# xingyizhou/CenterTrack

Hardware: NVIDIA H100
Metric: frames/sec (device-timed) DLA-34 512x512 (higher is better)
Workload: dtype bf16

## Files before the change

centertrack_b200/_lib.py:

```python
import ctypes as C
import os
import subprocess

_HERE = os.path.dirname(os.path.abspath(__file__))
LIB_PATH = os.path.join(_HERE, 'libctb200.so')
CSRC = os.path.join(_HERE, 'csrc')
SOURCES = ['api.cu', 'conv_simt.cu', 'conv_tc.cu', 'conv_halo.cu', 'elementwise.cu', 'decode.cu', 'stream.cu']

CT_F32, CT_BF16 = 0, 1
CT_A_CONV, CT_A_DCN, CT_A_DCN_WIN = 0, 1, 2
CT_OUT_NHWC, CT_OUT_NHWC_F32, CT_OUT_NCHW_F32, CT_OUT_NHWC_S2D = 0, 1, 2, 3
CT_HEAD_NONE, CT_HEAD_SIGMOID, CT_HEAD_DEPTH = 0, 1, 2
CT_ENGINE_SIMT, CT_ENGINE_TCGEN05, CT_ENGINE_TCGEN05_HALO, CT_ENGINE_TCGEN05_X3 = 0, 1, 2, 3
CT_ROLE_RAW, CT_ROLE_REG, CT_ROLE_WH, CT_ROLE_LTRB, CT_ROLE_LTRB_AMODAL, CT_ROLE_HPS = range(6)
CT_DECODE_MAX_HEADS = 12
CT_REC_SCORE, CT_REC_CLS, CT_REC_XS, CT_REC_YS, CT_REC_BBOX, CT_REC_IND, CT_REC_HEADS = 0, 1, 2, 3, 4, 8, 9


class ConvDesc(C.Structure):
  _fields_ = [
      ('engine', C.c_int32), ('dtype', C.c_int32), ('a_mode', C.c_int32),
      ('B', C.c_int32), ('H', C.c_int32), ('W', C.c_int32),
      ('C_in', C.c_int32), ('ld_in', C.c_int32), ('C_out', C.c_int32),
      ('KH', C.c_int32), ('KW', C.c_int32), ('stride', C.c_int32), ('pad', C.c_int32),
      ('OH', C.c_int32), ('OW', C.c_int32), ('ld_out', C.c_int32), ('out_mode', C.c_int32),
      ('relu', C.c_int32), ('ld_res', C.c_int32), ('head_act', C.c_int32),
      ('sig_from', C.c_int32), ('depth_scale', C.c_float), ('ld_om', C.c_int32),
      ('n_tile', C.c_int32), ('epilogue_sum3', C.c_int32), ('pad_w1', C.c_int32),
      ('x', C.c_void_p), ('w', C.c_void_p), ('shift', C.c_void_p), ('residual', C.c_void_p),
      ('om', C.c_void_p), ('out', C.c_void_p),
  ]


class DecodeHead(C.Structure):
  _fields_ = [('map', C.c_void_p), ('channels', C.c_int32), ('role', C.c_int32),
              ('rec_offset', C.c_int32)]


class DecodeDesc(C.Structure):
  _fields_ = [
# ... 19 lines not shown
      ('records', C.c_void_p), ('trans_out_inv', C.c_void_p), ('trans_input', C.c_void_p),
      ('tracks', C.c_void_p), ('counts', C.c_void_p), ('boxes', C.c_void_p),
  ]


class TrackAssoc(C.Structure):
  _fields_ = [
      ('hungarian', C.c_int32), ('public_det', C.c_int32), ('max_public', C.c_int32),
      ('public_ct', C.c_void_p), ('public_n', C.c_void_p), ('steps', C.c_void_p),
  ]


class TrackPayload(C.Structure):
  _fields_ = [
      ('width', C.c_int32), ('payload', C.c_void_p), ('rec_hps', C.c_int32), ('hps_floats', C.c_int32),
      ('rec_dep', C.c_int32), ('rec_dim', C.c_int32), ('rec_rot', C.c_int32), ('rec_amodel_offset', C.c_int32),
      ('rec_velocity', C.c_int32), ('velocity_floats', C.c_int32), ('rec_nuscenes_att', C.c_int32),
      ('att_floats', C.c_int32), ('calib', C.c_void_p),
  ]


EXPORTS = ['ct_packed_weight_bytes', 'ct_pack_weights', 'ct_conv_forward', 'ct_stem_forward',
           'ct_pack_stem_input', 'ct_pack_stem_input_f32', 'ct_maxpool2', 'ct_maxpool2_s2d', 'ct_upsample_add', 'ct_decode_workspace_bytes', 'ct_decode',
           'ct_render_pre_hm', 'ct_track_smem_bytes', 'ct_track_step', 'ct_track_assoc_smem_bytes',
           'ct_track_step_assoc', 'ct_track_payload_smem_bytes', 'ct_track_step_payload', 'ct_render_tracks', 'ct_flip_merge',
           'ct_warp_affine_normalize', 'ct_last_error', 'ct_abi_version', 'ct_launch_count',
           'ct_reset_launch_count', 'ct_debug_trace', 'ct_debug_watch']

NVCC_FLAGS = ['-gencode', 'arch=compute_90a,code=sm_90a', '-lineinfo', '-O3', '-std=c++17', '-Xcompiler', '-fPIC']


def build(force=False, verbose=False):
  srcs = [os.path.join(CSRC, s) for s in SOURCES]
  deps = srcs + [os.path.join(CSRC, h) for h in ('common.cuh', 'conv_common.cuh', 'ptx.cuh', 'wgmma.cuh')] + \
      [os.path.join(_HERE, '..', 'include', 'ctb200.h')]
  if not force and os.path.exists(LIB_PATH) and \
      all(os.path.getmtime(LIB_PATH) >= os.path.getmtime(d) for d in deps):
    return LIB_PATH
  import shutil
  import tempfile
  with tempfile.TemporaryDirectory(prefix='ctb_build_') as tmp:
    objs = [os.path.join(tmp, os.path.basename(s) + '.o') for s in srcs]
    procs = [subprocess.Popen(['nvcc'] + NVCC_FLAGS + (['-Xptxas', '-v'] if verbose else []) + ['-c', s, '-o', o],
                              stdout=subprocess.PIPE, stderr=subprocess.STDOUT, text=True)
             for s, o in zip(srcs, objs)]
    logs = [p.communicate()[0] for p in procs]
    for s, p, log in zip(srcs, procs, logs):
      if p.returncode != 0:
        raise RuntimeError('nvcc failed on %s:\n%s' % (os.path.basename(s), log))
    if verbose:
      print(''.join(logs))
    tmp_lib = os.path.join(tmp, 'libctb200.so')
    r = subprocess.run(['nvcc', '-gencode', 'arch=compute_90a,code=sm_90a', '-shared', '-o', tmp_lib] + objs,
                       capture_output=True, text=True)
    if r.returncode != 0:
      raise RuntimeError('nvcc link failed:\n' + r.stdout + r.stderr)
    shutil.move(tmp_lib, LIB_PATH)
  return LIB_PATH


_lib = None


def lib():
  global _lib
  if _lib is not None:
    return _lib
# ... 56 lines not shown
```

centertrack_b200/csrc/api.cu:

```cuda
#include "conv_common.cuh"
#include <vector>

namespace ctb {
thread_local char g_err[512] = {0};
thread_local int64_t g_launches = 0;

static inline uint16_t f32_to_bf16_rn(float f) {
  uint32_t u;
  memcpy(&u, &f, 4);
  if ((u & 0x7fffffffu) > 0x7f800000u) return (uint16_t)((u >> 16) | 0x40);
  const uint32_t lsb = (u >> 16) & 1u;
  u += 0x7fffu + lsb;
  return (uint16_t)(u >> 16);
}
}

using namespace ctb;

extern "C" const char* ct_last_error(void) { return g_err; }
extern "C" int ct_abi_version(void) { return CTB200_ABI_VERSION; }
extern "C" int64_t ct_launch_count(void) { return g_launches; }
extern "C" void ct_reset_launch_count(void) { g_launches = 0; }
extern "C" int ct_debug_trace(void* device_buf) {
  const int r = halo_set_trace(device_buf);
  return r != CT_OK ? r : tc_set_trace(device_buf);
}
extern "C" int ct_debug_watch(void* mapped_host_buf) {
  int r = halo_set_watch(mapped_host_buf);
  if (r == CT_OK) r = tc_set_watch(mapped_host_buf);
  if (r == CT_OK) r = decode_set_watch(mapped_host_buf);
  return r;
}

static inline int tc_k_slices(int C_in, int KH, int KW) { return (KH * KW * C_in + 63) / 64; }

extern "C" int64_t ct_packed_weight_bytes(int32_t engine, int32_t C_out, int32_t C_in, int32_t KH,
                                          int32_t KW, int32_t n_tile) {
  if (engine == CT_ENGINE_SIMT) {
    const int64_t ldw = (C_out + 63) / 64 * 64;
    return (int64_t)KH * KW * C_in * ldw * 4;
  }
  if (n_tile <= 0 || n_tile % 16 != 0 || n_tile > 256) return -1;
  const int64_t n_tiles = (C_out + n_tile - 1) / n_tile;
  if (engine == CT_ENGINE_TCGEN05_HALO) {
    if (!(C_in == 8 || (C_in % 16 == 0 && C_in <= 64) || (C_in % 64 == 0 && C_in <= 256))) return -1;
    return n_tiles * halo_blocks(C_in, KH, KW) * (int64_t)n_tile * 32;
  }
  return n_tiles * tc_k_slices(C_in, KH, KW) * (int64_t)n_tile * 64 * 2 * (engine == CT_ENGINE_TCGEN05_X3 ? 2 : 1);
}

extern "C" int ct_pack_weights(int32_t engine, const float* w, int32_t C_out, int32_t C_in, int32_t KH,
                               int32_t KW, int32_t n_tile, void* dst) {
  CT_REQUIRE(w && dst, "null pointer");
  CT_REQUIRE(C_out > 0 && C_in > 0 && KH > 0 && KW > 0, "bad shape");
  const int taps = KH * KW;
  if (engine == CT_ENGINE_SIMT) {
    const int ldw = (C_out + 63) / 64 * 64;
    float* o = (float*)dst;
    memset(o, 0, (size_t)taps * C_in * ldw * 4);
    for (int oc = 0; oc < C_out; ++oc)
      for (int c = 0; c < C_in; ++c)
        for (int t = 0; t < taps; ++t)
          o[((size_t)t * C_in + c) * ldw + oc] = w[((size_t)oc * C_in + c) * taps + t];
// ... 88 lines not shown
```

centertrack_b200/csrc/conv_common.cuh:

```cuda
#pragma once
#include "common.cuh"
#include <cudaTypedefs.h>
#include <type_traits>

namespace ctb {

struct ConvGeom {
  int B, H, W, C_in, ld_in;
  int C_out, KH, KW, stride, pad, pad_w, OH, OW;
  int ld_out, out_mode, relu, ld_res, head_act, sig_from;
  float depth_scale;
  int ld_om;
  int P_out;
  int K_total;
};

inline ConvGeom make_geom(const ct_conv_desc* d) {
  ConvGeom g;
  g.B = d->B; g.H = d->H; g.W = d->W; g.C_in = d->C_in; g.ld_in = d->ld_in;
  g.C_out = d->C_out; g.KH = d->KH; g.KW = d->KW; g.stride = d->stride; g.pad = d->pad;
  g.pad_w = d->pad_w1 > 0 ? d->pad_w1 - 1 : d->pad;
  g.OH = d->OH; g.OW = d->OW; g.ld_out = d->ld_out; g.out_mode = d->out_mode;
  g.relu = d->relu; g.ld_res = d->ld_res; g.head_act = d->head_act; g.sig_from = d->sig_from;
  g.depth_scale = d->depth_scale; g.ld_om = d->ld_om;
// ... 43 lines not shown
                    q == cudaDriverEntryPointSuccess;
    return ok ? reinterpret_cast<PFN_cuTensorMapEncodeTiled>(p) : nullptr;
  }();
  if (!encode) return fail(CT_ERR_CUDA, "cuTensorMapEncodeTiled entry point unavailable%s", "");
  const cuuint32_t estr[5] = {1, 1, 1, 1, 1};
  const CUresult cr = encode(map, CU_TENSOR_MAP_DATA_TYPE_BFLOAT16, (cuuint32_t)rank, const_cast<void*>(ptr), dims,
                             strides, box, estr, CU_TENSOR_MAP_INTERLEAVE_NONE, swizzle,
                             CU_TENSOR_MAP_L2_PROMOTION_L2_128B, CU_TENSOR_MAP_FLOAT_OOB_FILL_NONE);
  return cr == CUDA_SUCCESS ? CT_OK : fail(CT_ERR_CUDA, "cuTensorMapEncodeTiled failed%s (%ld)", "", (long)cr);
}

template <auto Kernel, typename... Args>
int launch_big_smem(dim3 grid, dim3 block, size_t smem, cudaStream_t st, const Args&... args) {
  int dev = 0;
  cudaGetDevice(&dev);
  static thread_local unsigned long long attr_set_mask = 0;
  if (dev >= 64 || !((attr_set_mask >> dev) & 1ull)) {
    CT_CUDA_OK(cudaFuncSetAttribute(Kernel, cudaFuncAttributeMaxDynamicSharedMemorySize, 227 * 1024));
    if (dev < 64) attr_set_mask |= 1ull << dev;
  }
  CT_CUDA_OK(launch_kernel(Kernel, grid, block, smem, st, true, args...));
  return after_launch();
}

template <int N = 16, typename F>
int dispatch_n_tile(int n_tile, F&& f) {
  if constexpr (N > 256) return fail(CT_ERR_INVALID, "unsupported n_tile%s (%ld)", "", (long)n_tile);
  else return n_tile == N ? f(std::integral_constant<int, N>()) : dispatch_n_tile<N + 16>(n_tile, f);
}

int conv_forward_simt(const ct_conv_desc* d, cudaStream_t st);
int conv_forward_tc(const ct_conv_desc* d, cudaStream_t st);
int conv_forward_halo(const ct_conv_desc* d, cudaStream_t st);
int halo_blocks(int C_in, int KH, int KW);
int halo_set_trace(void* buf);
int tc_set_trace(void* buf);
int halo_set_watch(void* mapped_host_buf);
int tc_set_watch(void* mapped_host_buf);
int decode_set_watch(void* mapped_host_buf);

}
```

centertrack_b200/csrc/conv_tc.cu:

```cuda
#include "conv_common.cuh"
#include "wgmma.cuh"
#include <cuda.h>
#include <stdlib.h>

namespace ctb {

constexpr int TC_BM = 128;
constexpr int TC_BK = 64;
constexpr int TC_THREADS = 256;
constexpr int TC_PRODUCERS = 256;
constexpr int TC_NROW = TC_BM * 8 / TC_PRODUCERS;
constexpr int A_STAGE_BYTES = TC_BM * 128;

struct TcArgs {
  ConvGeom g;
  const __nv_bfloat16* x;
  const __nv_bfloat16* w;
  const float* shift;
  const __nv_bfloat16* residual;
  const float* om;
  void* out;
  int n_tile, k_slices, stages, a_mode;
  int tiles_x, tiles_y;
  int win_m, win_pw, win_ph;
  uint32_t win_bytes;
  uint32_t region0;
};

struct __align__(16) DcnWinEntry { int goff; uint32_t meta; uint32_t w01, w23; };
constexpr uint32_t WIN_DX = 1u << 16, WIN_DY = 1u << 17, WIN_IN = 1u << 18;

__device__ __forceinline__ int tc_pixel(const TcArgs& a, int mt, int r) {
  const ConvGeom& g = a.g;
  if (a.tiles_x == 0) { const int p = mt * TC_BM + r; return p < g.P_out ? p : g.P_out; }
  const int tpi = a.tiles_x * a.tiles_y;
  const int b = mt / tpi, t = mt - b * tpi;
  const int ty = t / a.tiles_x, tx = t - ty * a.tiles_x;
  const int oy = ty * 8 + (r >> 4), ox = tx * 16 + (r & 15);
  return (oy < g.OH && ox < g.OW) ? (b * g.OH + oy) * g.OW + ox : g.P_out;
}

__device__ unsigned long long* g_tc_trace = nullptr;
__device__ __forceinline__ unsigned long long* tc_trace_ptr() {
  unsigned long long* t = g_tc_trace;
  return (t != nullptr && blockIdx.x == gridDim.x / 2 && blockIdx.y == 0) ? t : nullptr;
}
__device__ __forceinline__ void tc_stamp(unsigned long long* t, int k) {
  if (t != nullptr && k < 256) t[k] = (unsigned long long)clock64();
}

__device__ __forceinline__ uint64_t make_sdesc(uint32_t smem_addr) {
  return wg_desc(smem_addr, 16u, 1024u, 1u);
}

struct __align__(16) DcnEntry { int off, dxo, dyo, pad; float w00, w01, w10, w11; };

struct DcnCorner { int y0, x0, yc, xc; bool dx, dy; float w00, w01, w10, w11; };
__device__ __forceinline__ bool dcn_corner(float py, float px, int H, int W, float m, DcnCorner& c) {
  if (!(py > -1.f && py < (float)H && px > -1.f && px < (float)W)) return false;
  const float y0f = floorf(py), x0f = floorf(px);
  const int y0 = (int)y0f, x0 = (int)x0f;
  const float ly = py - y0f, lx = px - x0f, hy = 1.f - ly, hx = 1.f - lx;
  const bool y0ok = y0 >= 0, y1ok = y0 + 1 <= H - 1, x0ok = x0 >= 0, x1ok = x0 + 1 <= W - 1;
  c.y0 = y0; c.x0 = x0; c.yc = max(y0, 0); c.xc = max(x0, 0);
  c.dx = x0ok && x1ok; c.dy = y0ok && y1ok;
  c.w00 = (y0ok && x0ok) ? hy * hx * m : 0.f;
  c.w01 = (y0ok && x1ok) ? hy * lx * m : 0.f;
  c.w10 = (y1ok && x0ok) ? ly * hx * m : 0.f;
  c.w11 = (y1ok && x1ok) ? ly * lx * m : 0.f;
  return true;
}

__device__ __forceinline__ uint32_t bmul2(uint32_t a, uint32_t b) {
  uint32_t d;
  asm("mul.rn.bf16x2 %0, %1, %2;" : "=r"(d) : "r"(a), "r"(b));
  return d;
}
__device__ __forceinline__ uint32_t bfma2(uint32_t a, uint32_t b, uint32_t c) {
  uint32_t d;
  asm("fma.rn.bf16x2 %0, %1, %2, %3;" : "=r"(d) : "r"(a), "r"(b), "r"(c));
  return d;
}
__device__ __forceinline__ uint32_t dup_bf2(float w) {
  uint32_t d;
  asm("cvt.rn.bf16x2.f32 %0, %1, %1;" : "=r"(d) : "f"(w));
  return d;
}

__device__ __forceinline__ void split8(const float4 lo4, const float4 hi4, uint4& h, uint4& l) {
  const float f[8] = {lo4.x, lo4.y, lo4.z, lo4.w, hi4.x, hi4.y, hi4.z, hi4.w};
  uint32_t hh[4], ll[4];
#pragma unroll
  for (int q = 0; q < 4; ++q) {
    const __nv_bfloat162 hp = __floats2bfloat162_rn(f[2 * q], f[2 * q + 1]);
    const float2 hf = __bfloat1622float2(hp);
    const __nv_bfloat162 lp = __floats2bfloat162_rn(f[2 * q] - hf.x, f[2 * q + 1] - hf.y);
    hh[q] = *reinterpret_cast<const uint32_t*>(&hp);
    ll[q] = *reinterpret_cast<const uint32_t*>(&lp);
  }
  h = make_uint4(hh[0], hh[1], hh[2], hh[3]);
  l = make_uint4(ll[0], ll[1], ll[2], ll[3]);
}
template <bool X3, int N>
__global__ void __launch_bounds__(TC_THREADS, (!X3 && N <= 64) ? 2 : 1)
conv_tc_kernel(const TcArgs a, const __grid_constant__ CUtensorMap tmap) {
  extern __shared__ __align__(1024) unsigned char smem_dyn[];
  unsigned char* smem = smem_dyn + ((1024u - (smem_u32(smem_dyn) & 1023u)) & 1023u);
  const ConvGeom& g = a.g;
  const int tid = threadIdx.x, warp = tid >> 5, lane = tid & 31;
  const int wg = tid >> 7;
  unsigned long long* const trace = tc_trace_ptr();
  const int S = a.stages;
  constexpr uint32_t b_tile_bytes = (uint32_t)N * 128u;
  constexpr uint32_t b_stage_bytes = X3 ? 2u * b_tile_bytes : b_tile_bytes;
  constexpr uint32_t a_stage_bytes = X3 ? 2u * A_STAGE_BYTES : A_STAGE_BYTES;
// ... 190 lines not shown
      for (int k = 0; k < TC_BK / 16; ++k) {
        Wgmma<N>::mma(acc, ad_lo + 2ull * k, bd + 2ull * k, (s > 0 || k > 0) ? 1u : 0u);
        Wgmma<N>::mma(acc, ad + 2ull * k, bd_lo + 2ull * k, 1u);
        Wgmma<N>::mma(acc, ad + 2ull * k, bd + 2ull * k, 1u);
      }
    } else {
#pragma unroll
      for (int k = 0; k < TC_BK / 16; ++k)
        Wgmma<N>::mma(acc, ad + 2ull * k, bd + 2ull * k, (s > 0 || k > 0) ? 1u : 0u);
    }
    wg_commit();
    wg_wait<1>();
    wg_fence_operand(acc);
    if (s > 0) {
      __syncwarp();
      if (lane == 0) mbar_arrive(empty_bar((s - 1) % S));
    }
  };

  if (win) {
    const int nchunks = g.C_in >> 6;
    const uint32_t pitch = (uint32_t)a.win_pw * 128u;
    const int gdx = g.ld_in, gdy = g.W * g.ld_in;
    int s = 0;
    for (int ch = 0; ch < nchunks; ++ch) {
      mbar_wait(win_bar, (uint32_t)ch & 1u);
      for (int tap = 0; tap < 9; ++tap, ++s) {
        const int stage = begin_stage(s);
        const DcnWinEntry* tab = win_tab + tap * TC_BM + rb;
        uint4 e4[TC_NROW], v[TC_NROW][4];
#pragma unroll
        for (int i = 0; i < TC_NROW; ++i) e4[i] = *reinterpret_cast<const uint4*>(&tab[16 * i]);
#pragma unroll
        for (int i = 0; i < TC_NROW; ++i) {
          const uint32_t meta = e4[i].y;
          if (meta & WIN_IN) {
            const uint32_t base = s_win + ((meta & 0xffffu) << 4) + (uint32_t)(q << 4);
            const uint32_t dx = (meta & WIN_DX) ? 128u : 0u, dy = (meta & WIN_DY) ? pitch : 0u;
            v[i][0] = lds16(base); v[i][1] = lds16(base + dx);
            v[i][2] = lds16(base + dy); v[i][3] = lds16(base + dy + dx);
          } else {
            const __nv_bfloat16* p00 = a.x + ((int)e4[i].x + (ch << 6) + (q << 3));
            const int dx = (meta & WIN_DX) ? gdx : 0, dy = (meta & WIN_DY) ? gdy : 0;
            v[i][0] = ldg_nc16(p00); v[i][1] = ldg_nc16(p00 + dx);
            v[i][2] = ldg_nc16(p00 + dy); v[i][3] = ldg_nc16(p00 + dy + dx);
          }
        }
        const uint32_t dst = sA + stage * A_STAGE_BYTES + (uint32_t)rb * 128u + swz;
#pragma unroll
        for (int i = 0; i < TC_NROW; ++i) {
          const uint32_t w0 = __byte_perm(e4[i].z, 0, 0x1010), w1 = __byte_perm(e4[i].z, 0, 0x3232);
          const uint32_t w2 = __byte_perm(e4[i].w, 0, 0x1010), w3 = __byte_perm(e4[i].w, 0, 0x3232);
          uint4 o;
          o.x = bmul2(v[i][0].x, w0); o.y = bmul2(v[i][0].y, w0); o.z = bmul2(v[i][0].z, w0); o.w = bmul2(v[i][0].w, w0);
          o.x = bfma2(v[i][1].x, w1, o.x); o.y = bfma2(v[i][1].y, w1, o.y); o.z = bfma2(v[i][1].z, w1, o.z); o.w = bfma2(v[i][1].w, w1, o.w);
          o.x = bfma2(v[i][2].x, w2, o.x); o.y = bfma2(v[i][2].y, w2, o.y); o.z = bfma2(v[i][2].z, w2, o.z); o.w = bfma2(v[i][2].w, w2, o.w);
          o.x = bfma2(v[i][3].x, w3, o.x); o.y = bfma2(v[i][3].y, w3, o.y); o.z = bfma2(v[i][3].z, w3, o.z); o.w = bfma2(v[i][3].w, w3, o.w);
          sts16(dst + i * 2048u, o);
        }
        end_stage(s, stage);
      }
      if (ch + 1 < nchunks) {
        named_sync(1, TC_PRODUCERS);
        if (tid == 0) {
          mbar_arrive_expect_tx(win_bar, a.win_bytes);
          tma_4d(s_win, &tmap, (ch + 1) << 6, win_x0, win_y0, win_b, win_bar);
        }
      }
    }
  } else if constexpr (X3) {
    if (a.a_mode == CT_A_DCN) {
      float4 va[2][4][2], vb[2][4][2];
      auto load_half = [&](int tap, int c, int half, float4 (&v)[2][4][2]) {
        const DcnEntry* tab = dcn_tab + (tap < ntaps ? tap : 0) * TC_BM + rb + 32 * half;
#pragma unroll
        for (int j = 0; j < 2; ++j) {
          const int4 o = *reinterpret_cast<const int4*>(&tab[16 * j]);
          const float* p00 = xf + (o.x + c);
          v[j][0][0] = ldg_nc_f4(p00);             v[j][0][1] = ldg_nc_f4(p00 + 4);
          v[j][1][0] = ldg_nc_f4(p00 + o.y);       v[j][1][1] = ldg_nc_f4(p00 + o.y + 4);
          v[j][2][0] = ldg_nc_f4(p00 + o.z);       v[j][2][1] = ldg_nc_f4(p00 + o.z + 4);
          v[j][3][0] = ldg_nc_f4(p00 + o.z + o.y); v[j][3][1] = ldg_nc_f4(p00 + o.z + o.y + 4);
        }
      };
      auto blend_half = [&](int tap, int stage, int half, const float4 (&v)[2][4][2]) {
        const bool live = tap < ntaps;
        const DcnEntry* tab = dcn_tab + (live ? tap : 0) * TC_BM + rb + 32 * half;
        const uint32_t dst = sA + stage * a_stage_bytes + (uint32_t)(rb + 32 * half) * 128u + swz;
#pragma unroll
        for (int j = 0; j < 2; ++j) {
          const float4 w = *reinterpret_cast<const float4*>(&tab[16 * j].w00);
          const float ww[4] = {w.x, w.y, w.z, w.w};
// ... 261 lines not shown
  }
  if (win) {
    static const int win_stages = getenv("CTB_TC_WIN_STAGES") ? atoi(getenv("CTB_TC_WIN_STAGES")) : 0;
    stages = 2;
    if (win_stages >= 2) stages = win_stages;
  }
  while (stages > 2 && smem_for(stages) > 227 * 1024) --stages;
  if (smem_for(stages) > 227 * 1024)
    return fail(CT_ERR_UNSUPPORTED, "conv_tc: tile does not fit in shared memory%s (%ld)", "", (long)smem_for(stages));
  if (stages > a.k_slices) stages = a.k_slices;
  a.stages = stages;
  a.region0 = (uint32_t)region0_for(stages);
  const size_t smem = smem_for(stages);
  const int n_tiles = (g.C_out + n_tile - 1) / n_tile;
  static const int tile2d_env = getenv("CTB_TC_TILE2D") ? atoi(getenv("CTB_TC_TILE2D")) : 0;
  a.tiles_x = a.tiles_y = 0;
  int m_tiles = (g.P_out + TC_BM - 1) / TC_BM;
  if (tile2d_env && g.OW % 16 == 0 && g.OH % 8 == 0) {
    a.tiles_x = g.OW / 16;
    a.tiles_y = g.OH / 8;
    m_tiles = g.B * a.tiles_x * a.tiles_y;
  }
  CUtensorMap tmap;
  memset(&tmap, 0, sizeof(tmap));
  if (win) {
    a.tiles_x = (g.OW + 15) / 16;
    a.tiles_y = (g.OH + 7) / 8;
    m_tiles = g.B * a.tiles_x * a.tiles_y;
    const cuuint64_t dims[4] = {(cuuint64_t)g.C_in, (cuuint64_t)g.W, (cuuint64_t)g.H, (cuuint64_t)g.B};
    const cuuint64_t strides[3] = {(cuuint64_t)g.ld_in * 2, (cuuint64_t)g.W * g.ld_in * 2, (cuuint64_t)g.H * g.W * g.ld_in * 2};
    const cuuint32_t box[4] = {64, (cuuint32_t)a.win_pw, (cuuint32_t)a.win_ph, 1};
    const int r = encode_tmap_bf16(&tmap, d->x, 4, dims, strides, box, CU_TENSOR_MAP_SWIZZLE_NONE);
    if (r != CT_OK) return r;
  }
  dim3 grid(m_tiles, n_tiles);
  return dispatch_n_tile(n_tile, [&](auto n) {
    constexpr int N = decltype(n)::value;
    return x3 ? launch_big_smem<conv_tc_kernel<true, N>>(grid, dim3(TC_THREADS), smem, st, a, tmap)
              : launch_big_smem<conv_tc_kernel<false, N>>(grid, dim3(TC_THREADS), smem, st, a, tmap);
  });
}

}
```

Before: 2124.

## Add warp-specialized persistent DCN window kernel with table, sampler and MMA warps

Adds a persistent, warp-specialized kernel for windowed deformable convolution and makes it the default (CTB_DCN_WS=1) for NHWC outputs. Dedicated warps each do one job: build the bilinear sampling table, TMA-load the input windows, load weights, blend samples into A tiles, and run wgmma. They hand off through mbarrier pipelines, with setmaxnreg rebalancing registers between roles. The aim is to overlap offset/mask table construction and sampling with tensor-core work and to hide per-tile setup. The cost is more complex synchronization, heavier shared-memory use, and a grid capped at the SM count.

After: 2160, median of 6. +1.7%, better.

```diff
diff --git a/centertrack_b200/_lib.py b/centertrack_b200/_lib.py
--- a/centertrack_b200/_lib.py
+++ b/centertrack_b200/_lib.py
@@ -5,7 +5,7 @@
 _HERE = os.path.dirname(os.path.abspath(__file__))
 LIB_PATH = os.path.join(_HERE, 'libctb200.so')
 CSRC = os.path.join(_HERE, 'csrc')
-SOURCES = ['api.cu', 'conv_simt.cu', 'conv_tc.cu', 'conv_halo.cu', 'elementwise.cu', 'decode.cu', 'stream.cu']
+SOURCES = ['api.cu', 'conv_simt.cu', 'conv_tc.cu', 'conv_dcn.cu', 'conv_halo.cu', 'elementwise.cu', 'decode.cu', 'stream.cu']
 
 CT_F32, CT_BF16 = 0, 1
 CT_A_CONV, CT_A_DCN, CT_A_DCN_WIN = 0, 1, 2
@@ -91,7 +91,7 @@
 
 def build(force=False, verbose=False):
   srcs = [os.path.join(CSRC, s) for s in SOURCES]
-  deps = srcs + [os.path.join(CSRC, h) for h in ('common.cuh', 'conv_common.cuh', 'ptx.cuh', 'wgmma.cuh')] + \
+  deps = srcs + [os.path.join(CSRC, h) for h in ('common.cuh', 'conv_common.cuh', 'dcn_win.cuh', 'ptx.cuh', 'wgmma.cuh')] + \
       [os.path.join(_HERE, '..', 'include', 'ctb200.h')]
   if not force and os.path.exists(LIB_PATH) and \
       all(os.path.getmtime(LIB_PATH) >= os.path.getmtime(d) for d in deps):
diff --git a/centertrack_b200/csrc/api.cu b/centertrack_b200/csrc/api.cu
--- a/centertrack_b200/csrc/api.cu
+++ b/centertrack_b200/csrc/api.cu
@@ -22,13 +22,16 @@
 extern "C" int64_t ct_launch_count(void) { return g_launches; }
 extern "C" void ct_reset_launch_count(void) { g_launches = 0; }
 extern "C" int ct_debug_trace(void* device_buf) {
-  const int r = halo_set_trace(device_buf);
-  return r != CT_OK ? r : tc_set_trace(device_buf);
+  int r = halo_set_trace(device_buf);
+  if (r == CT_OK) r = tc_set_trace(device_buf);
+  if (r == CT_OK) r = dcn_set_trace(device_buf);
+  return r;
 }
 extern "C" int ct_debug_watch(void* mapped_host_buf) {
   int r = halo_set_watch(mapped_host_buf);
   if (r == CT_OK) r = tc_set_watch(mapped_host_buf);
   if (r == CT_OK) r = decode_set_watch(mapped_host_buf);
+  if (r == CT_OK) r = dcn_set_watch(mapped_host_buf);
   return r;
 }
 
diff --git a/centertrack_b200/csrc/conv_common.cuh b/centertrack_b200/csrc/conv_common.cuh
--- a/centertrack_b200/csrc/conv_common.cuh
+++ b/centertrack_b200/csrc/conv_common.cuh
@@ -99,11 +99,15 @@
 int conv_forward_simt(const ct_conv_desc* d, cudaStream_t st);
 int conv_forward_tc(const ct_conv_desc* d, cudaStream_t st);
 int conv_forward_halo(const ct_conv_desc* d, cudaStream_t st);
+int conv_forward_dcn_ws(const ct_conv_desc* d, int win_m, const CUtensorMap& tmap, cudaStream_t st);
+size_t dcn_ws_smem_bytes(int n_tile, uint32_t win_bytes);
 int halo_blocks(int C_in, int KH, int KW);
 int halo_set_trace(void* buf);
 int tc_set_trace(void* buf);
 int halo_set_watch(void* mapped_host_buf);
 int tc_set_watch(void* mapped_host_buf);
 int decode_set_watch(void* mapped_host_buf);
+int dcn_set_watch(void* mapped_host_buf);
+int dcn_set_trace(void* buf);
 
 }
diff --git a/centertrack_b200/csrc/conv_dcn.cu b/centertrack_b200/csrc/conv_dcn.cu
--- /dev/null
+++ b/centertrack_b200/csrc/conv_dcn.cu
@@ -0,0 +1,334 @@
+#include "dcn_win.cuh"
+#include "wgmma.cuh"
+#include <cuda.h>
+#include <stdlib.h>
+
+namespace ctb {
+
+constexpr int DW_BM = 128;
+constexpr int DW_SA = 3;
+constexpr uint32_t DW_A_BYTES = DW_BM * 128;
+constexpr uint32_t DW_TAB_BYTES = 9 * DW_BM * sizeof(DcnWinEntry);
+constexpr uint32_t DW_STG_BYTES = 64 * EPI_PITCH * 4;
+
+template <int N>
+struct DwCfg {
+  static constexpr int SB = N == 64 ? 3 : 2;
+  static constexpr uint32_t B_BYTES = (uint32_t)N * 128u;
+  static constexpr int SW = 8;
+  static constexpr int THREADS = (8 + SW + 4) * 32;
+  static constexpr int REG_LAUNCH = 96;
+  static constexpr int REG_CONSUMER = N == 64 ? 96 : 112;
+  static constexpr int REG_SAMPLER = N == 64 ? 104 : 88;
+  static constexpr int REG_TABLE = 80;
+};
+
+struct DcnWsArgs {
+  ConvGeom g;
+  const __nv_bfloat16* x;
+  const __nv_bfloat16* w;
+  const float* shift;
+  const __nv_bfloat16* residual;
+  const float* om;
+  __nv_bfloat16* out;
+  int tiles_x, tiles_y, n_tiles, items, nchunks, k_slices;
+  int win_m, win_pw, win_ph;
+  uint32_t win_bytes, win_stride;
+};
+
+__device__ unsigned long long* g_dw_trace = nullptr;
+__device__ __forceinline__ unsigned long long* dw_trace_ptr() {
+  unsigned long long* t = g_dw_trace;
+  return (t != nullptr && blockIdx.x == gridDim.x / 2) ? t : nullptr;
+}
+__device__ __forceinline__ void dw_stamp(unsigned long long* t, int j, int k) {
+  if (t != nullptr && j < 32) t[8 * j + k] = (unsigned long long)clock64();
+}
+
+template <int R>
+__device__ __forceinline__ void reg_alloc() { asm volatile("setmaxnreg.inc.sync.aligned.u32 %0;" ::"n"(R)); }
+template <int R>
+__device__ __forceinline__ void reg_dealloc() { asm volatile("setmaxnreg.dec.sync.aligned.u32 %0;" ::"n"(R)); }
+
+template <int N>
+__host__ __device__ inline uint32_t dw_smem_layout(uint32_t win_stride, uint32_t* off_win, uint32_t* off_tab,
+                                                   uint32_t* off_stg, uint32_t* off_bar) {
+  const uint32_t b = DW_SA * DW_A_BYTES;
+  *off_win = b + DwCfg<N>::SB * DwCfg<N>::B_BYTES;
+  *off_tab = *off_win + 2u * win_stride;
+  *off_stg = *off_tab + 2u * DW_TAB_BYTES;
+  *off_bar = *off_stg + 2u * DW_STG_BYTES;
+  return *off_bar + 256u;
+}
+
+template <int N>
+__global__ void __launch_bounds__(DwCfg<N>::THREADS, 1)
+dcn_win_kernel(const DcnWsArgs a, const __grid_constant__ CUtensorMap tmap) {
+  extern __shared__ __align__(1024) unsigned char dsm_dyn[];
+  unsigned char* sm = dsm_dyn + ((1024u - (smem_u32(dsm_dyn) & 1023u)) & 1023u);
+  using Cfg = DwCfg<N>;
+  constexpr int SB = Cfg::SB, SW = Cfg::SW;
+  constexpr int W_TABLE = 8 + SW, W_LOADER = 8 + SW + 3;
+  const ConvGeom& g = a.g;
+  const int tid = threadIdx.x, warp = tid >> 5, lane = tid & 31;
+  unsigned long long* const trace = dw_trace_ptr();
+  uint32_t off_win, off_tab, off_stg, off_bar;
+  dw_smem_layout<N>(a.win_stride, &off_win, &off_tab, &off_stg, &off_bar);
+  const uint32_t base = smem_u32(sm);
+  const uint32_t sA = base, sB = base + DW_SA * DW_A_BYTES, sWin = base + off_win;
+  DcnWinEntry* const tabs = reinterpret_cast<DcnWinEntry*>(sm + off_tab);
+  const uint32_t bars = base + off_bar;
+  auto tab_full = [&](int i) { return bars + 8u * i; };
+  auto tab_empty = [&](int i) { return bars + 8u * (2 + i); };
+  auto win_full = [&](int i) { return bars + 8u * (4 + i); };
+  auto win_empty = [&](int i) { return bars + 8u * (6 + i); };
+  auto a_full = [&](int i) { return bars + 8u * (8 + i); };
+  auto a_empty = [&](int i) { return bars + 8u * (8 + DW_SA + i); };
+  auto b_full = [&](int i) { return bars + 8u * (8 + 2 * DW_SA + i); };
+  auto b_empty = [&](int i) { return bars + 8u * (8 + 2 * DW_SA + SB + i); };
+
+  pdl_trigger();
+  if (tid == 0) {
+    for (int i = 0; i < 2; ++i) {
+      mbar_init(tab_full(i), 3); mbar_init(tab_empty(i), SW);
+      mbar_init(win_full(i), 1); mbar_init(win_empty(i), SW);
+    }
+    for (int i = 0; i < DW_SA; ++i) { mbar_init(a_full(i), SW); mbar_init(a_empty(i), 8); }
+    for (int i = 0; i < SB; ++i) { mbar_init(b_full(i), 1); mbar_init(b_empty(i), 8); }
+    mbar_init_fence();
+  }
+  __syncthreads();
+
+  const int KS = a.k_slices;
+  const int tpi = a.tiles_x * a.tiles_y;
+
+  if constexpr (Cfg::REG_TABLE < Cfg::REG_LAUNCH)
+    if (warp >= W_TABLE) reg_dealloc<Cfg::REG_TABLE>();
+  if (warp == W_LOADER) {
+    if (lane == 0) {
+      uint32_t gs = 0;
+      for (int it = blockIdx.x; it < a.items; it += gridDim.x) {
+        const __nv_bfloat16* wt = a.w + (size_t)(it % a.n_tiles) * KS * N * 64;
+        for (int s = 0; s < KS; ++s, ++gs) {
+          const int st = gs % SB;
+          mbar_wait(b_empty(st), ((gs / SB) & 1u) ^ 1u, 20, gs);
+          mbar_arrive_expect_tx(b_full(st), Cfg::B_BYTES);
+          bulk_g2s(sB + st * Cfg::B_BYTES, wt + (size_t)s * N * 64, Cfg::B_BYTES, b_full(st));
+        }
+      }
+    }
+  } else if (warp >= W_TABLE) {
+    pdl_wait();
+    const int t0 = tid - W_TABLE * 32;
+    uint32_t gc = 0;
+    int j = 0;
+    for (int it = blockIdx.x; it < a.items; it += gridDim.x, ++j) {
+      const int tb = j & 1;
+      mbar_wait(tab_empty(tb), (((uint32_t)j >> 1) & 1u) ^ 1u, 21, j);
+      const int mt = it / a.n_tiles;
+      const int b = mt / tpi, t = mt - b * tpi;
+      const int ty = t / a.tiles_x, tx = t - ty * a.tiles_x;
+      const int win_y0 = ty * 8 - 1 - a.win_m, win_x0 = tx * 16 - 1 - a.win_m;
+      auto load_window = [&](int c) {
+        const int wb = gc & 1;
+        mbar_wait(win_empty(wb), ((gc >> 1) & 1u) ^ 1u, 22, gc);
+        mbar_arrive_expect_tx(win_full(wb), a.win_bytes);
+        tma_4d(sWin + wb * a.win_stride, &tmap, c << 6, win_x0, win_y0, b, win_full(wb));
+        ++gc;
+      };
+      if (t0 == 0) load_window(0);
+      const int img = b * g.H * g.W;
+      DcnWinEntry* tab = tabs + tb * 9 * DW_BM;
+      for (int trow = t0; trow < DW_BM; trow += 96) {
+        const int oy = ty * 8 + (trow >> 4), ox = tx * 16 + (trow & 15);
+        const bool ok = oy < g.OH && ox < g.OW;
+        float om[28];
+#pragma unroll
+        for (int k = 0; k < 28; ++k) om[k] = 0.f;
+        if (ok) {
+          const float4* omp = reinterpret_cast<const float4*>(a.om + ((size_t)(b * g.OH + oy) * g.OW + ox) * g.ld_om);
+#pragma unroll
+          for (int k = 0; k < 7; ++k) {
+            const float4 t4 = __ldg(omp + k);
+            om[4 * k] = t4.x; om[4 * k + 1] = t4.y; om[4 * k + 2] = t4.z; om[4 * k + 3] = t4.w;
+          }
+        }
+#pragma unroll
+        for (int tap = 0; tap < 9; ++tap)
+          tab[tap * DW_BM + trow] = dcn_win_entry(ok, oy, ox, img, tap, om[2 * tap], om[2 * tap + 1], om[18 + tap], g,
+                                                  win_y0, win_x0, a.win_ph, a.win_pw);
+      }
+      __syncwarp();
+      if (lane == 0) mbar_arrive(tab_full(tb));
+      if (t0 == 0) dw_stamp(trace, j, 0);
+      if (t0 == 0)
+        for (int c = 1; c < a.nchunks; ++c) load_window(c);
+    }
+  } else if (warp >= 8) {
+    if constexpr (Cfg::REG_SAMPLER > Cfg::REG_LAUNCH) reg_alloc<Cfg::REG_SAMPLER>();
+    else if constexpr (Cfg::REG_SAMPLER < Cfg::REG_LAUNCH) reg_dealloc<Cfg::REG_SAMPLER>();
+    pdl_wait();
+    constexpr int RG = SW * 4;
+    constexpr int NR = DW_BM / RG;
+    const int st = tid - 256;
+    const int q = st & 7;
+    const int rb = st >> 3;
+    const uint32_t swz = (uint32_t)((q ^ (rb & 7)) << 4);
+    const uint32_t pitch = (uint32_t)a.win_pw * 128u;
+    const int gdx = g.ld_in, gdy = g.W * g.ld_in;
+    uint32_t gs = 0, gc = 0;
+    int j = 0;
+    for (int it = blockIdx.x; it < a.items; it += gridDim.x, ++j) {
+      const int tb = j & 1;
+      mbar_wait(tab_full(tb), ((uint32_t)j >> 1) & 1u, 23, j);
+      if (st == 0) dw_stamp(trace, j, 1);
+      unsigned long long stall = 0;
+      const DcnWinEntry* tab = tabs + tb * 9 * DW_BM + rb;
+      for (int ch = 0; ch < a.nchunks; ++ch, ++gc) {
+        const int wb = gc & 1;
+        mbar_wait(win_full(wb), (gc >> 1) & 1u, 24, gc);
+        const uint32_t s_win = sWin + wb * a.win_stride;
+        for (int tap = 0; tap < 9; ++tap, ++gs) {
+          const int stage = gs % DW_SA;
+          uint4 e4[NR], v[NR][4];
+#pragma unroll
+          for (int i = 0; i < NR; ++i) e4[i] = *reinterpret_cast<const uint4*>(&tab[tap * DW_BM + RG * i]);
+#pragma unroll
+          for (int i = 0; i < NR; ++i) dcn_win_load(e4[i], s_win, pitch, q, a.x, ch << 6, gdx, gdy, v[i]);
+          const unsigned long long w0 = trace != nullptr ? clock64() : 0ull;
+          mbar_wait(a_empty(stage), ((gs / DW_SA) & 1u) ^ 1u, 25, gs);
+          if (trace != nullptr) stall += clock64() - w0;
+          const uint32_t dst = sA + stage * DW_A_BYTES + (uint32_t)rb * 128u + swz;
+#pragma unroll
+          for (int i = 0; i < NR; ++i) sts16(dst + i * (RG * 128u), dcn_win_blend(e4[i], v[i]));
+          fence_proxy_async();
+          __syncwarp();
+          if (lane == 0) mbar_arrive(a_full(stage));
+          if (st == 0 && ch == 0 && tap == 0) dw_stamp(trace, j, 2);
+        }
+        __syncwarp();
+        if (lane == 0) mbar_arrive(win_empty(wb));
+      }
+      __syncwarp();
+      if (lane == 0) mbar_arrive(tab_empty(tb));
+      if (st == 0) {
+        dw_stamp(trace, j, 3);
+        if (trace != nullptr && j < 32) trace[8 * j + 7] = stall;
+      }
+    }
+  } else {
+    if constexpr (Cfg::REG_CONSUMER > Cfg::REG_LAUNCH) reg_alloc<Cfg::REG_CONSUMER>();
+    pdl_wait();
+    const int wg = warp >> 2, w4 = warp & 3;
+    const int lrow = 32 * (w4 & 1) + lane;
+    const int chalf = w4 >> 1;
+    const int row = 64 * wg + lrow;
+    const uint32_t stg = base + off_stg + (uint32_t)wg * DW_STG_BYTES;
+    float acc[N / 2];
+#pragma unroll
+    for (int i = 0; i < N / 2; ++i) acc[i] = 0.f;
+    uint32_t gs = 0;
+    int j = 0;
+    for (int it = blockIdx.x; it < a.items; it += gridDim.x, ++j) {
+      for (int s = 0; s < KS; ++s, ++gs) {
+        const int sa = gs % DW_SA, sb = gs % SB;
+        mbar_wait(a_full(sa), (gs / DW_SA) & 1u, 26, gs);
+        mbar_wait(b_full(sb), (gs / SB) & 1u, 27, gs);
+        if (tid == 0 && s == 0) dw_stamp(trace, j, 4);
+        const uint64_t ad = wg_desc(sA + sa * DW_A_BYTES + (uint32_t)wg * (64u * 128u), 16u, 1024u, 1u);
+        const uint64_t bd = wg_desc(sB + sb * Cfg::B_BYTES, 16u, 1024u, 1u);
+        wg_fence();
+#pragma unroll
+        for (int k = 0; k < 4; ++k) Wgmma<N>::mma(acc, ad + 2ull * k, bd + 2ull * k, (s > 0 || k > 0) ? 1u : 0u);
+        wg_commit();
+        wg_wait<1>();
+        wg_fence_operand(acc);
+        if (s > 0) {
+          __syncwarp();
+          if (lane == 0) { mbar_arrive(a_empty((gs - 1) % DW_SA)); mbar_arrive(b_empty((gs - 1) % SB)); }
+        }
+      }
+      wg_wait<0>();
+      wg_fence_operand(acc);
+      if (tid == 0) dw_stamp(trace, j, 5);
+      __syncwarp();
+      if (lane == 0) { mbar_arrive(a_empty((gs - 1) % DW_SA)); mbar_arrive(b_empty((gs - 1) % SB)); }
+
+      const int mt = it / a.n_tiles, n0 = (it - mt * a.n_tiles) * N;
+      const int b = mt / tpi, t = mt - b * tpi;
+      const int ty = t / a.tiles_x, tx = t - ty * a.tiles_x;
+      const int oy = ty * 8 + (row >> 4), ox = tx * 16 + (row & 15);
+      const bool p_ok = oy < g.OH && ox < g.OW;
+      const size_t p = ((size_t)b * g.OH + oy) * g.OW + ox;
+#pragma unroll
+      for (int c0 = 0; c0 < N; c0 += 32) {
+        named_sync(1 + wg, 128);
+        stage_acc_chunk(acc, c0, stg, 0);
+        named_sync(1 + wg, 128);
+        const int o0 = n0 + c0 + chalf * 16;
+        if (!p_ok || o0 >= g.C_out) continue;
+        float v[16];
+        lds_f(stg + ((uint32_t)lrow * EPI_PITCH + (uint32_t)chalf * 16u) * 4u, v);
+        if (a.shift) {
+#pragma unroll
+          for (int k = 0; k < 16; ++k) v[k] += __ldg(a.shift + o0 + k);
+        }
+        if (a.residual) {
+          const uint4* rp = reinterpret_cast<const uint4*>(a.residual + p * g.ld_res + o0);
+          add_residual_bf16(v, ldg_nc16(rp), ldg_nc16(rp + 1));
+        }
+        relu16(v, g.relu);
+        store_bf16x16(a.out + p * g.ld_out + o0, v);
+      }
+      if (tid == 0) dw_stamp(trace, j, 6);
+    }
+  }
+}
+
+int dcn_set_watch(void* mapped_host_buf) { return set_mbar_watch(mapped_host_buf); }
+int dcn_set_trace(void* buf) {
+  unsigned long long* p = (unsigned long long*)buf;
+  return cudaMemcpyToSymbol(g_dw_trace, &p, sizeof(p)) == cudaSuccess ? CT_OK : CT_ERR_CUDA;
+}
+
+static uint32_t dw_win_stride(uint32_t win_bytes) { return (win_bytes + 127u) & ~127u; }
+
+size_t dcn_ws_smem_bytes(int n_tile, uint32_t win_bytes) {
+  uint32_t ow, ot, os, ob;
+  const uint32_t ws = dw_win_stride(win_bytes);
+  if (n_tile == 64) return dw_smem_layout<64>(ws, &ow, &ot, &os, &ob) + 1024;
+  if (n_tile == 128) return dw_smem_layout<128>(ws, &ow, &ot, &os, &ob) + 1024;
+  return ~(size_t)0;
+}
+
+int conv_forward_dcn_ws(const ct_conv_desc* d, int win_m, const CUtensorMap& tmap, cudaStream_t st) {
+  DcnWsArgs a;
+  a.g = make_geom(d);
+  const ConvGeom& g = a.g;
+  a.x = (const __nv_bfloat16*)d->x;
+  a.w = (const __nv_bfloat16*)d->w;
+  a.shift = d->shift;
+  a.residual = (const __nv_bfloat16*)d->residual;
+  a.om = d->om;
+  a.out = (__nv_bfloat16*)d->out;
+  a.tiles_x = (g.OW + 15) / 16;
+  a.tiles_y = (g.OH + 7) / 8;
+  a.n_tiles = (g.C_out + d->n_tile - 1) / d->n_tile;
+  a.items = g.B * a.tiles_x * a.tiles_y * a.n_tiles;
+  a.nchunks = g.C_in / 64;
+  a.k_slices = 9 * a.nchunks;
+  a.win_m = win_m;
+  a.win_pw = 16 + 2 * win_m + 3;
+  a.win_ph = 8 + 2 * win_m + 3;
+  a.win_bytes = (uint32_t)(a.win_pw * a.win_ph * 128);
+  a.win_stride = dw_win_stride(a.win_bytes);
+  const size_t smem = dcn_ws_smem_bytes(d->n_tile, a.win_bytes);
+  if (smem > 227 * 1024)
+    return fail(CT_ERR_UNSUPPORTED, "dcn_win_kernel: tile does not fit in shared memory%s (%ld)", "", (long)smem);
+  const int sms = device_sm_count();
+  const dim3 grid(a.items < sms ? a.items : sms);
+  if (d->n_tile == 64) return launch_big_smem<dcn_win_kernel<64>>(grid, dim3(DwCfg<64>::THREADS), smem, st, a, tmap);
+  return launch_big_smem<dcn_win_kernel<128>>(grid, dim3(DwCfg<128>::THREADS), smem, st, a, tmap);
+}
+
+}
diff --git a/centertrack_b200/csrc/conv_tc.cu b/centertrack_b200/csrc/conv_tc.cu
--- a/centertrack_b200/csrc/conv_tc.cu
+++ b/centertrack_b200/csrc/conv_tc.cu
@@ -1,4 +1,5 @@
 #include "conv_common.cuh"
+#include "dcn_win.cuh"
 #include "wgmma.cuh"
 #include <cuda.h>
 #include <stdlib.h>
@@ -27,9 +28,6 @@
   uint32_t region0;
 };
 
-struct __align__(16) DcnWinEntry { int goff; uint32_t meta; uint32_t w01, w23; };
-constexpr uint32_t WIN_DX = 1u << 16, WIN_DY = 1u << 17, WIN_IN = 1u << 18;
-
 __device__ __forceinline__ int tc_pixel(const TcArgs& a, int mt, int r) {
   const ConvGeom& g = a.g;
   if (a.tiles_x == 0) { const int p = mt * TC_BM + r; return p < g.P_out ? p : g.P_out; }
@@ -55,32 +53,6 @@
 
 struct __align__(16) DcnEntry { int off, dxo, dyo, pad; float w00, w01, w10, w11; };
 
-struct DcnCorner { int y0, x0, yc, xc; bool dx, dy; float w00, w01, w10, w11; };
-__device__ __forceinline__ bool dcn_corner(float py, float px, int H, int W, float m, DcnCorner& c) {
-  if (!(py > -1.f && py < (float)H && px > -1.f && px < (float)W)) return false;
-  const float y0f = floorf(py), x0f = floorf(px);
-  const int y0 = (int)y0f, x0 = (int)x0f;
-  const float ly = py - y0f, lx = px - x0f, hy = 1.f - ly, hx = 1.f - lx;
-  const bool y0ok = y0 >= 0, y1ok = y0 + 1 <= H - 1, x0ok = x0 >= 0, x1ok = x0 + 1 <= W - 1;
-  c.y0 = y0; c.x0 = x0; c.yc = max(y0, 0); c.xc = max(x0, 0);
-  c.dx = x0ok && x1ok; c.dy = y0ok && y1ok;
-  c.w00 = (y0ok && x0ok) ? hy * hx * m : 0.f;
-  c.w01 = (y0ok && x1ok) ? hy * lx * m : 0.f;
-  c.w10 = (y1ok && x0ok) ? ly * hx * m : 0.f;
-  c.w11 = (y1ok && x1ok) ? ly * lx * m : 0.f;
-  return true;
-}
-
-__device__ __forceinline__ uint32_t bmul2(uint32_t a, uint32_t b) {
-  uint32_t d;
-  asm("mul.rn.bf16x2 %0, %1, %2;" : "=r"(d) : "r"(a), "r"(b));
-  return d;
-}
-__device__ __forceinline__ uint32_t bfma2(uint32_t a, uint32_t b, uint32_t c) {
-  uint32_t d;
-  asm("fma.rn.bf16x2 %0, %1, %2, %3;" : "=r"(d) : "r"(a), "r"(b), "r"(c));
-  return d;
-}
 __device__ __forceinline__ uint32_t dup_bf2(float w) {
   uint32_t d;
   asm("cvt.rn.bf16x2.f32 %0, %1, %1;" : "=r"(d) : "f"(w));
@@ -337,32 +309,10 @@
 #pragma unroll
         for (int i = 0; i < TC_NROW; ++i) e4[i] = *reinterpret_cast<const uint4*>(&tab[16 * i]);
 #pragma unroll
-        for (int i = 0; i < TC_NROW; ++i) {
-          const uint32_t meta = e4[i].y;
-          if (meta & WIN_IN) {
-            const uint32_t base = s_win + ((meta & 0xffffu) << 4) + (uint32_t)(q << 4);
-            const uint32_t dx = (meta & WIN_DX) ? 128u : 0u, dy = (meta & WIN_DY) ? pitch : 0u;
-            v[i][0] = lds16(base); v[i][1] = lds16(base + dx);
-            v[i][2] = lds16(base + dy); v[i][3] = lds16(base + dy + dx);
-          } else {
-            const __nv_bfloat16* p00 = a.x + ((int)e4[i].x + (ch << 6) + (q << 3));
-            const int dx = (meta & WIN_DX) ? gdx : 0, dy = (meta & WIN_DY) ? gdy : 0;
-            v[i][0] = ldg_nc16(p00); v[i][1] = ldg_nc16(p00 + dx);
-            v[i][2] = ldg_nc16(p00 + dy); v[i][3] = ldg_nc16(p00 + dy + dx);
-          }
-        }
+        for (int i = 0; i < TC_NROW; ++i) dcn_win_load(e4[i], s_win, pitch, q, a.x, ch << 6, gdx, gdy, v[i]);
         const uint32_t dst = sA + stage * A_STAGE_BYTES + (uint32_t)rb * 128u + swz;
 #pragma unroll
-        for (int i = 0; i < TC_NROW; ++i) {
-          const uint32_t w0 = __byte_perm(e4[i].z, 0, 0x1010), w1 = __byte_perm(e4[i].z, 0, 0x3232);
-          const uint32_t w2 = __byte_perm(e4[i].w, 0, 0x1010), w3 = __byte_perm(e4[i].w, 0, 0x3232);
-          uint4 o;
-          o.x = bmul2(v[i][0].x, w0); o.y = bmul2(v[i][0].y, w0); o.z = bmul2(v[i][0].z, w0); o.w = bmul2(v[i][0].w, w0);
-          o.x = bfma2(v[i][1].x, w1, o.x); o.y = bfma2(v[i][1].y, w1, o.y); o.z = bfma2(v[i][1].z, w1, o.z); o.w = bfma2(v[i][1].w, w1, o.w);
-          o.x = bfma2(v[i][2].x, w2, o.x); o.y = bfma2(v[i][2].y, w2, o.y); o.z = bfma2(v[i][2].z, w2, o.z); o.w = bfma2(v[i][2].w, w2, o.w);
-          o.x = bfma2(v[i][3].x, w3, o.x); o.y = bfma2(v[i][3].y, w3, o.y); o.z = bfma2(v[i][3].z, w3, o.z); o.w = bfma2(v[i][3].w, w3, o.w);
-          sts16(dst + i * 2048u, o);
-        }
+        for (int i = 0; i < TC_NROW; ++i) sts16(dst + i * 2048u, dcn_win_blend(e4[i], v[i]));
         end_stage(s, stage);
       }
       if (ch + 1 < nchunks) {
@@ -690,6 +640,10 @@
     const cuuint32_t box[4] = {64, (cuuint32_t)a.win_pw, (cuuint32_t)a.win_ph, 1};
     const int r = encode_tmap_bf16(&tmap, d->x, 4, dims, strides, box, CU_TENSOR_MAP_SWIZZLE_NONE);
     if (r != CT_OK) return r;
+    static const int dcn_ws_env = getenv("CTB_DCN_WS") ? atoi(getenv("CTB_DCN_WS")) : 1;
+    if (dcn_ws_env && (n_tile == 64 || n_tile == 128) && g.out_mode == CT_OUT_NHWC &&
+        dcn_ws_smem_bytes(n_tile, a.win_bytes) <= 227 * 1024)
+      return conv_forward_dcn_ws(d, a.win_m, tmap, st);
   }
   dim3 grid(m_tiles, n_tiles);
   return dispatch_n_tile(n_tile, [&](auto n) {
diff --git a/centertrack_b200/csrc/dcn_win.cuh b/centertrack_b200/csrc/dcn_win.cuh
--- /dev/null
+++ b/centertrack_b200/csrc/dcn_win.cuh
@@ -0,0 +1,82 @@
+#pragma once
+#include "conv_common.cuh"
+#include "ptx.cuh"
+
+namespace ctb {
+
+struct DcnCorner { int y0, x0, yc, xc; bool dx, dy; float w00, w01, w10, w11; };
+__device__ __forceinline__ bool dcn_corner(float py, float px, int H, int W, float m, DcnCorner& c) {
+  if (!(py > -1.f && py < (float)H && px > -1.f && px < (float)W)) return false;
+  const float y0f = floorf(py), x0f = floorf(px);
+  const int y0 = (int)y0f, x0 = (int)x0f;
+  const float ly = py - y0f, lx = px - x0f, hy = 1.f - ly, hx = 1.f - lx;
+  const bool y0ok = y0 >= 0, y1ok = y0 + 1 <= H - 1, x0ok = x0 >= 0, x1ok = x0 + 1 <= W - 1;
+  c.y0 = y0; c.x0 = x0; c.yc = max(y0, 0); c.xc = max(x0, 0);
+  c.dx = x0ok && x1ok; c.dy = y0ok && y1ok;
+  c.w00 = (y0ok && x0ok) ? hy * hx * m : 0.f;
+  c.w01 = (y0ok && x1ok) ? hy * lx * m : 0.f;
+  c.w10 = (y1ok && x0ok) ? ly * hx * m : 0.f;
+  c.w11 = (y1ok && x1ok) ? ly * lx * m : 0.f;
+  return true;
+}
+
+__device__ __forceinline__ uint32_t bmul2(uint32_t a, uint32_t b) {
+  uint32_t d;
+  asm("mul.rn.bf16x2 %0, %1, %2;" : "=r"(d) : "r"(a), "r"(b));
+  return d;
+}
+__device__ __forceinline__ uint32_t bfma2(uint32_t a, uint32_t b, uint32_t c) {
+  uint32_t d;
+  asm("fma.rn.bf16x2 %0, %1, %2, %3;" : "=r"(d) : "r"(a), "r"(b), "r"(c));
+  return d;
+}
+
+struct __align__(16) DcnWinEntry { int goff; uint32_t meta; uint32_t w01, w23; };
+constexpr uint32_t WIN_DX = 1u << 16, WIN_DY = 1u << 17, WIN_IN = 1u << 18;
+
+__device__ __forceinline__ DcnWinEntry dcn_win_entry(bool ok, int oy, int ox, int img, int tap, float dy, float dx,
+                                                     float m, const ConvGeom& g, int win_y0, int win_x0, int win_ph,
+                                                     int win_pw) {
+  DcnWinEntry e; e.goff = 0; e.meta = WIN_IN; e.w01 = 0u; e.w23 = 0u;
+  DcnCorner c;
+  if (ok && dcn_corner((float)(oy - 1 + tap / 3) + dy, (float)(ox - 1 + tap % 3) + dx, g.H, g.W, m, c)) {
+    e.goff = (img + c.yc * g.W + c.xc) * g.ld_in;
+    const bool inside = c.y0 >= win_y0 && c.y0 + 1 <= win_y0 + win_ph - 1 && c.x0 >= win_x0 &&
+                        c.x0 + 1 <= win_x0 + win_pw - 1;
+    const uint32_t woff16 = (uint32_t)((c.yc - win_y0) * win_pw + (c.xc - win_x0)) * 8u;
+    e.meta = (inside ? (woff16 | WIN_IN) : 0u) | (c.dx ? WIN_DX : 0u) | (c.dy ? WIN_DY : 0u);
+    const __nv_bfloat162 wa = __floats2bfloat162_rn(c.w00, c.w01), wb = __floats2bfloat162_rn(c.w10, c.w11);
+    e.w01 = *reinterpret_cast<const uint32_t*>(&wa);
+    e.w23 = *reinterpret_cast<const uint32_t*>(&wb);
+  }
+  return e;
+}
+
+__device__ __forceinline__ void dcn_win_load(const uint4 e, uint32_t s_win, uint32_t pitch, int q,
+                                             const __nv_bfloat16* x, int c0, int gdx, int gdy, uint4 (&v)[4]) {
+  const uint32_t meta = e.y;
+  if (meta & WIN_IN) {
+    const uint32_t base = s_win + ((meta & 0xffffu) << 4) + (uint32_t)(q << 4);
+    const uint32_t dx = (meta & WIN_DX) ? 128u : 0u, dy = (meta & WIN_DY) ? pitch : 0u;
+    v[0] = lds16(base); v[1] = lds16(base + dx);
+    v[2] = lds16(base + dy); v[3] = lds16(base + dy + dx);
+  } else {
+    const __nv_bfloat16* p00 = x + ((int)e.x + c0 + (q << 3));
+    const int dx = (meta & WIN_DX) ? gdx : 0, dy = (meta & WIN_DY) ? gdy : 0;
+    v[0] = ldg_nc16(p00); v[1] = ldg_nc16(p00 + dx);
+    v[2] = ldg_nc16(p00 + dy); v[3] = ldg_nc16(p00 + dy + dx);
+  }
+}
+
+__device__ __forceinline__ uint4 dcn_win_blend(const uint4 e, const uint4 (&v)[4]) {
+  const uint32_t w0 = __byte_perm(e.z, 0, 0x1010), w1 = __byte_perm(e.z, 0, 0x3232);
+  const uint32_t w2 = __byte_perm(e.w, 0, 0x1010), w3 = __byte_perm(e.w, 0, 0x3232);
+  uint4 o;
+  o.x = bmul2(v[0].x, w0); o.y = bmul2(v[0].y, w0); o.z = bmul2(v[0].z, w0); o.w = bmul2(v[0].w, w0);
+  o.x = bfma2(v[1].x, w1, o.x); o.y = bfma2(v[1].y, w1, o.y); o.z = bfma2(v[1].z, w1, o.z); o.w = bfma2(v[1].w, w1, o.w);
+  o.x = bfma2(v[2].x, w2, o.x); o.y = bfma2(v[2].y, w2, o.y); o.z = bfma2(v[2].z, w2, o.z); o.w = bfma2(v[2].w, w2, o.w);
+  o.x = bfma2(v[3].x, w3, o.x); o.y = bfma2(v[3].y, w3, o.y); o.z = bfma2(v[3].z, w3, o.z); o.w = bfma2(v[3].w, w3, o.w);
+  return o;
+}
+
+}
```
